# krea-ai/realtime-video

Hardware: AMD Instinct MI355X
Metric: frames/sec at 832x480, 4-step 14B T2V (per-step DiT latency in config) (higher is better)
Workload: dtype bf16

## Files before the change

realtime_video_amd/_lib.py:

```python
import ctypes
import os
import re
import subprocess

_HERE = os.path.dirname(os.path.abspath(__file__))
LIB_PATH = os.environ.get("RTV_LIB_PATH") or os.path.join(_HERE, "librtv_hip.so")
CSRC = os.path.join(_HERE, "csrc")

_INCLUDE = os.path.join(os.path.dirname(_HERE), "include")
HEADERS = ("rtv_hip.h", "rtv_hip_lab.h")

_lib = None

_SCALARS = {"int": ctypes.c_int, "int64_t": ctypes.c_int64, "float": ctypes.c_float, "double": ctypes.c_double,
            "size_t": ctypes.c_size_t}
_RETURNS = {"int": ctypes.c_int, "size_t": ctypes.c_size_t, "const char*": ctypes.c_char_p}
_STARS = r"(\*(?:\s*const\s*\*)?)?"


def _field_type(base, stars, structs):
    value = _SCALARS.get(base) or structs.get(base)
    if not stars:
        return value
    if base == "void":
        return ctypes.c_void_p if stars == "*" else ctypes.POINTER(ctypes.c_void_p)
    return ctypes.POINTER(value) if value and stars == "*" else None


def _param_type(base, stars, structs):
    if not stars:
        return ctypes.c_void_p if base == "rtv_stream_t" else _SCALARS.get(base)
    if base in structs:
        return ctypes.POINTER(structs[base]) if stars == "*" else None
    return ctypes.c_void_p if base == "void" or base in _SCALARS else None


def parse_header(text, structs):
    text = re.sub(r"/\*.*?\*/", "", text, flags=re.S)
    text = re.sub(r"#ifdef __cplusplus.*?#endif", "", text, flags=re.S)
    text = re.sub(r"^[ \t]*#.*$", "", text, flags=re.M)
    text = re.sub(r"\benum\s*\{[^}]*\}\s*;|\btypedef\s+void\s*\*\s*rtv_stream_t\s*;", "", text)

    def struct(m):
        name, fields = m.group(2), []
        for decl in filter(None, (d.strip() for d in m.group(1).split(";"))):
            head = re.match(r"(?:const\s+)?(\w+)\s*", decl)
            for item in decl[head.end():].split(","):
                d = re.fullmatch(_STARS + r"\s*(\w+)((?:\s*\[\d+\])*)", item.strip())
                t = d and _field_type(head.group(1), re.sub(r"\s", "", d.group(1) or ""), structs)
                if not t:
                    raise ValueError(f"{name}: cannot bind field declaration `{decl}`")
                for n in reversed(re.findall(r"\d+", d.group(3))):
                    t = t * int(n)
                fields.append((d.group(2), t))
        structs[name] = type(name, (ctypes.Structure,), {"_fields_": fields})
        return ""

    text = re.sub(r"\btypedef\s+struct\s*\w*\s*\{([^}]*)\}\s*(\w+)\s*;", struct, text)
    protos = {}
    for stmt in filter(None, (" ".join(s.split()) for s in text.split(";"))):
        m = re.fullmatch(r"(.*?)\s*\b(\w+)\s*\((.*)\)", stmt)
        if not m:
            raise ValueError(f"cannot bind declaration `{stmt}`")
        ret, name, params = m.group(1).replace(" *", "*"), m.group(2), m.group(3).strip()
        if ret not in _RETURNS:
            raise ValueError(f"{name}: cannot bind return type `{ret}`")
        argtypes = []
        for param in ([] if params == "void" else params.split(",")):
            d = re.fullmatch(r"(?:const\s+)?(\w+)\s*" + _STARS + r"\s*(\w+)?", param.strip())
            t = d and _param_type(d.group(1), re.sub(r"\s", "", d.group(2) or ""), structs)
            if not t:
                raise ValueError(f"{name}: cannot bind parameter `{param.strip()}`")
            argtypes.append(t)
        protos[name] = (_RETURNS[ret], argtypes)
    return protos


def _read(name):
    with open(os.path.join(_INCLUDE, name)) as f:
        return f.read()


STRUCTS, PROTOTYPES = {}, {}
for _name in HEADERS:
    PROTOTYPES.update(parse_header(_read(_name), STRUCTS))
IO_HEADER = "rtv_hip_io.h"
IO_STRUCTS = dict(STRUCTS)
IO_PROTOTYPES = parse_header(_read(IO_HEADER), IO_STRUCTS)
IO_STRUCTS = {k: v for k, v in IO_STRUCTS.items() if k not in STRUCTS}
JPEG_HEADER = "rtv_hip_jpeg.h"
JPEG_STRUCTS = dict(STRUCTS)
JPEG_PROTOTYPES = parse_header(_read(JPEG_HEADER), JPEG_STRUCTS)
JPEG_STRUCTS = {k: v for k, v in JPEG_STRUCTS.items() if k not in STRUCTS}
JPEGDEC_HEADER = "rtv_hip_jpeg_decode.h"
JPEGDEC_STRUCTS = dict(STRUCTS)
JPEGDEC_PROTOTYPES = parse_header(_read(JPEGDEC_HEADER), JPEGDEC_STRUCTS)
JPEGDEC_STRUCTS = {k: v for k, v in JPEGDEC_STRUCTS.items() if k not in STRUCTS}
LORA_HEADER = "rtv_hip_lora.h"
LORA_STRUCTS = dict(STRUCTS)
LORA_PROTOTYPES = parse_header(_read(LORA_HEADER), LORA_STRUCTS)
LORA_STRUCTS = {k: v for k, v in LORA_STRUCTS.items() if k not in STRUCTS}
CROSS_FOLD_HEADER = "rtv_hip_cross_fold.h"
CROSS_FOLD_STRUCTS = dict(STRUCTS)
CROSS_FOLD_PROTOTYPES = parse_header(_read(CROSS_FOLD_HEADER), CROSS_FOLD_STRUCTS)
FP8_ROWS_HEADER = "rtv_hip_fp8_rows.h"
FP8_ROWS_PROTOTYPES = parse_header(_read(FP8_ROWS_HEADER), dict(STRUCTS))
ATTN_FP8_HEADER = "rtv_hip_attn_fp8.h"
ATTN_FP8_STRUCTS = dict(STRUCTS)
ATTN_FP8_PROTOTYPES = parse_header(_read(ATTN_FP8_HEADER), ATTN_FP8_STRUCTS)
ATTN_FP8_STRUCTS = {k: v for k, v in ATTN_FP8_STRUCTS.items() if k not in STRUCTS}
MXFP4_HEADER = "rtv_hip_mxfp4.h"
MXFP4_PROTOTYPES = parse_header(_read(MXFP4_HEADER), dict(STRUCTS))
MXFP6_HEADER = "rtv_hip_mxfp6.h"
MXFP6_PROTOTYPES = parse_header(_read(MXFP6_HEADER), dict(STRUCTS))
MX_ROTATE_HEADER = "rtv_hip_mx_rotate.h"
MX_ROTATE_PROTOTYPES = parse_header(_read(MX_ROTATE_HEADER), dict(STRUCTS))
MX_ROT_ACT_SHIFT, MX_ROT_WEIGHT_SHIFT, MX_ROT_MAX_SHIFT = (
    int(re.search(rf"^#define\s+RTV_MX_ROT_{n}_SHIFT\s+(\d+)", _read(MX_ROTATE_HEADER), flags=re.M).group(1)) for n in ("ACT", "WEIGHT", "MAX"))
LORA_MAX_ADAPTERS, LORA_MAX_RANK = (int(re.search(rf"^#define\s+RTV_LORA_MAX_{n}\s+(\d+)", _read(LORA_HEADER), flags=re.M).group(1))
                                    for n in ("ADAPTERS", "RANK"))
FRAMES_MAX = int(re.search(r"^#define\s+RTV_FRAMES_MAX\s+(\d+)", _read(IO_HEADER), flags=re.M).group(1))
ABI_VERSION = int(re.search(r"^#define\s+RTV_ABI_VERSION\s+(\d+)", _read(HEADERS[0]), flags=re.M).group(1))


def build(verbose=False):
    jobs = os.environ.get("MAX_JOBS") or str(min(16, len(os.sched_getaffinity(0)) if hasattr(os, "sched_getaffinity") else os.cpu_count() or 4))
    cmd = ["make", "-C", CSRC, "-j", jobs]
    res = subprocess.run(cmd, capture_output=True, text=True)
    if verbose or res.returncode != 0:
        print(res.stdout[-4000:])
        print(res.stderr[-4000:])
    if res.returncode != 0:
        raise RuntimeError("building librtv_hip.so failed")
    return LIB_PATH


def declared_symbols(lab=True):
    out = set()
    for name in HEADERS if lab else HEADERS[:1]:
        text = re.sub(r"/\*.*?\*/", "", _read(name), flags=re.S)
        out.update(re.findall(r"\b(rtv_[a-z0-9_]+)\s*\(", text))
    return sorted(out)


def load():
    global _lib
    if _lib is not None:
        return _lib
    if not os.path.exists(LIB_PATH):
        raise RuntimeError(
            f"{LIB_PATH} is missing: run `python -c 'import __graft_entry__ as g; g.build()'` "
            "(or `make -C realtime_video_amd/csrc`). There is no CPU fallback for the HIP path.")
    lib = ctypes.CDLL(LIB_PATH)
    for name, (restype, argtypes) in list(PROTOTYPES.items()) + list(IO_PROTOTYPES.items()) + list(JPEG_PROTOTYPES.items()) + list(JPEGDEC_PROTOTYPES.items()) + list(LORA_PROTOTYPES.items()) + list(CROSS_FOLD_PROTOTYPES.items()) + list(FP8_ROWS_PROTOTYPES.items()) + list(ATTN_FP8_PROTOTYPES.items()) + list(MXFP4_PROTOTYPES.items()) + list(MXFP6_PROTOTYPES.items()) + list(MX_ROTATE_PROTOTYPES.items()):
        fn = getattr(lib, name, None)
        if fn is None:
            if os.environ.get("RTV_LIB_PATH"):
                continue
            raise RuntimeError(f"librtv_hip.so does not export {name}")
        fn.restype, fn.argtypes = restype, argtypes
    have = lib.rtv_version()
    if have != ABI_VERSION:
        raise RuntimeError(f"{LIB_PATH} reports ABI revision {have}, include/rtv_hip.h declares RTV_ABI_VERSION {ABI_VERSION}: "
                           "rebuild the library (`make -C realtime_video_amd/csrc`)")
    _lib = lib
    return lib


def check(status, what):
    if status != 0:
        msg = load().rtv_last_error().decode("utf-8", "replace")
        raise RuntimeError(f"{what} failed (status {status}): {msg}")


def call(name, *args):
    check(getattr(load(), name)(*args), name)
```

realtime_video_amd/csrc/vae_decode.hip:

```cpp
#include "gemm_core.h"
#include "rtv_internal.h"

namespace rtv {

struct ConvParams;
int launch_conv(const ConvParams& p, hipStream_t stream);

constexpr int RN_CHUNKS = 3;
__global__ __launch_bounds__(256) void rmsnorm_silu_cl_kernel(const f16_t* __restrict__ x, f16_t* __restrict__ out,
                                                             const f16_t* __restrict__ gamma, int C,
                                                             int64_t npix, int apply_silu) {
  __shared__ float ssq[64];
  __shared__ float part[256 * RN_CHUNKS];
  const int G = C >> 3;
  const int ppb = (256 * RN_CHUNKS) / G;
  const int64_t pix0 = (int64_t)blockIdx.x * ppb;
  float v[RN_CHUNKS][8];
  int lp[RN_CHUNKS];
#pragma unroll
  for (int i = 0; i < RN_CHUNKS; ++i) {
    const int c = threadIdx.x + i * 256;
    lp[i] = c / G;
    const int64_t pix = pix0 + lp[i];
    float s = 0.f;
    if (pix < npix) {
      u32x4 raw = *(const u32x4*)(x + pix * C + (c - lp[i] * G) * 8);
#pragma unroll
      for (int j = 0; j < 4; ++j) {
        const uint32_t u = raw[j];
        unpack_f16x2(u, v[i][2 * j], v[i][2 * j + 1]);
        s += v[i][2 * j] * v[i][2 * j] + v[i][2 * j + 1] * v[i][2 * j + 1];
      }
    }
    part[c] = s;
  }
  __syncthreads();
  if ((int)threadIdx.x < ppb) {
    float t = 0.f;
    for (int k = 0; k < G; ++k) t += part[threadIdx.x * G + k];
    ssq[threadIdx.x] = t;
  }
  __syncthreads();
  const float sqrtC = sqrtf((float)C);
#pragma unroll
  for (int i = 0; i < RN_CHUNKS; ++i) {
    const int c = threadIdx.x + i * 256;
    const int64_t pix = pix0 + lp[i];
    if (pix < npix) {
      const int ch = (c - lp[i] * G) * 8;
      const float inv = sqrtC / fmaxf(sqrtf(ssq[lp[i]]), 1e-12f);
      u32x4 graw = *(const u32x4*)(gamma + ch);
      u32x4 o;
#pragma unroll
      for (int j = 0; j < 4; ++j) {
        const uint32_t gu = graw[j];
        float g0, g1;
        unpack_f16x2(gu, g0, g1);
        float a = v[i][2 * j] * inv * g0;
        float b = v[i][2 * j + 1] * inv * g1;
        if (apply_silu) {
          a = silu(a);
          b = silu(b);
        }
        o[j] = pack_f16x2(a, b);
      }
      *(u32x4*)(out + pix * C + ch) = o;
    }
  }
}

__global__ __launch_bounds__(256) void softmax_rows_kernel(const f16_t* __restrict__ s, int lds_, f16_t* __restrict__ p,
                                                          int ldp, int n) {
  __shared__ float red[8];
  const int row = blockIdx.x;
  const f16_t* sr = s + (size_t)row * lds_;
  f16_t* pr = p + (size_t)row * ldp;
  float mx = -INFINITY;
  for (int c = threadIdx.x * 8; c < n; c += 256 * 8) {
    u32x4 raw = *(const u32x4*)(sr + c);
#pragma unroll
    for (int j = 0; j < 4; ++j) {
      const uint32_t u = raw[j];
      float a, b;
      unpack_f16x2(u, a, b);
      mx = fmaxf(mx, fmaxf(a, b));
    }
  }
  mx = wave_max(mx);
  if ((threadIdx.x & 63) == 0) red[threadIdx.x >> 6] = mx;
  __syncthreads();
  mx = fmaxf(fmaxf(red[0], red[1]), fmaxf(red[2], red[3]));
  float sum = 0.f;
  for (int c = threadIdx.x * 8; c < n; c += 256 * 8) {
    u32x4 raw = *(const u32x4*)(sr + c);
#pragma unroll
    for (int j = 0; j < 4; ++j) {
      const uint32_t u = raw[j];
      float a, b;
      unpack_f16x2(u, a, b);
      sum += __expf(a - mx) + __expf(b - mx);
    }
  }
  sum = wave_sum(sum);
  __syncthreads();
  if ((threadIdx.x & 63) == 0) red[4 + (threadIdx.x >> 6)] = sum;
  __syncthreads();
  const float inv = 1.0f / (red[4] + red[5] + red[6] + red[7]);
  for (int c = threadIdx.x * 8; c < ldp; c += 256 * 8) {
    u32x4 o = {0u, 0u, 0u, 0u};
    if (c < n) {
      u32x4 raw = *(const u32x4*)(sr + c);
#pragma unroll
      for (int j = 0; j < 4; ++j) {
        const uint32_t u = raw[j];
        float a, b;
        unpack_f16x2(u, a, b);
        o[j] = pack_f16x2(__expf(a - mx) * inv, __expf(b - mx) * inv);
      }
    }
    *(u32x4*)(pr + c) = o;
  }
}

__global__ void upsample_cache_t1_kernel(f16_t* buf, int64_t slice) {
  for (int64_t i = (int64_t)blockIdx.x * blockDim.x + threadIdx.x; i < slice; i += (int64_t)gridDim.x * blockDim.x) {
    f16_t c1 = buf[slice + i], x = buf[2 * slice + i];
    buf[i] = ((c1 & 0x7fff) == 0) ? (f16_t)0 : x;
    buf[slice + i] = x;
  }
}

__global__ void vae_prep_kernel(const f16_t* __restrict__ z, int t, int hw, const float* __restrict__ mean,
                                const float* __restrict__ stdv, const float* __restrict__ w2 ,
                                const float* __restrict__ b2, f16_t* __restrict__ out) {
  const int p = blockIdx.x * blockDim.x + threadIdx.x;
  if (p >= hw) return;
  float zin[16];
#pragma unroll
  for (int c = 0; c < 16; ++c) {
    float zz = f16_to_f32(z[((size_t)t * 16 + c) * hw + p]);
    float inv = round_f16(1.0f / round_f16(stdv[c]));
    zin[c] = round_f16(round_f16(zz / inv) + round_f16(mean[c]));
  }
  u32x4 o[4];
#pragma unroll
  for (int co = 0; co < 16; co += 2) {
    float a = b2[co], b = b2[co + 1];
#pragma unroll
    for (int c = 0; c < 16; ++c) {
      a += w2[co * 16 + c] * zin[c];
      b += w2[(co + 1) * 16 + c] * zin[c];
    }
    o[co >> 3][(co & 7) >> 1] = pack_f16x2(a, b);
  }
  o[2] = u32x4{0u, 0u, 0u, 0u};
  o[3] = u32x4{0u, 0u, 0u, 0u};
  u32x4* dst = (u32x4*)(out + (size_t)p * 32);
  dst[0] = o[0];
  dst[1] = o[1];
  dst[2] = o[2];
  dst[3] = o[3];
}

__global__ void vae_final_kernel(const f16_t* __restrict__ in, float* __restrict__ out, int T, int64_t hw, int64_t in_hw,
                                 int64_t skip_px) {
  const int64_t total = (int64_t)T * hw;
  for (int64_t i = (int64_t)blockIdx.x * blockDim.x + threadIdx.x; i < total; i += (int64_t)gridDim.x * blockDim.x) {
    const int64_t t = i / hw, p = i - t * hw;
    u32x2 raw = *(const u32x2*)(in + (t * in_hw + skip_px + p) * 8);
    const uint32_t u0 = raw[0], u1 = raw[1];
    float c0, c1, c2, c3;
    unpack_f16x2(u0, c0, c1);
    unpack_f16x2(u1, c2, c3);
    float r = fminf(fmaxf(c0, -1.f), 1.f), g = fminf(fmaxf(c1, -1.f), 1.f), bl = fminf(fmaxf(c2, -1.f), 1.f);
    out[(t * 3 + 0) * hw + p] = r;
    out[(t * 3 + 1) * hw + p] = g;
    out[(t * 3 + 2) * hw + p] = bl;
  }
}

}

using namespace rtv;

extern "C" int rtv_conv_cl(const void* in, const void* w, const void* bias, const void* residual, int res_ld,
                           void* out, int out_ld, int T, int H, int W, int Cin, int Cout, int kt, int kh, int kw,
                           int resample, int n_split, const void* zeros, rtv_stream_t stream);

#define RTV_TRY(expr)       \
  do {                      \
    int _s = (expr);        \
    if (_s != 0) return _s; \
  } while (0)

extern "C" int rtv_rmsnorm_silu_cl(const void* x, void* out, const void* gamma, int C, int64_t npix, int apply_silu,
                                   rtv_stream_t stream) {
  if (npix <= 0) return 0;
  if (C % 8 || 768 % (C / 8) || (768 / (C / 8)) > 64) return set_error(-1, "rmsnorm_silu_cl: C must be 96, 192, 384 (or another divisor layout of 768 chunks)");
  const int ppb = 768 / (C / 8);
  ProfScope prof(PROF_LN, (hipStream_t)stream, 2.0 * npix * C * 2);
  hipLaunchKernelGGL(rmsnorm_silu_cl_kernel, dim3((unsigned)((npix + ppb - 1) / ppb)), dim3(256), 0,
                     (hipStream_t)stream, (const f16_t*)x, (f16_t*)out, (const f16_t*)gamma, C, npix, apply_silu);
  return check_launch("rmsnorm_silu_cl");
}

extern "C" int rtv_softmax_rows(const void* s, int lds_, void* p, int ldp, int rows, int n, rtv_stream_t stream) {
  if (rows <= 0) return 0;
  if (n % 8 || lds_ % 8 || ldp % 8 || ldp < n) return set_error(-1, "softmax_rows: n / strides must be multiples of 8");
  hipLaunchKernelGGL(softmax_rows_kernel, dim3(rows), dim3(256), 0, (hipStream_t)stream, (const f16_t*)s, lds_,
                     (f16_t*)p, ldp, n);
  return check_launch("softmax_rows");
}

namespace {

struct Stage {
  int H, W;
};

struct RowPlan {
  int a[4], b[4];
  int r0, r1;
};

static int make_plan(int h, int r0, int r1, RowPlan* P) {
  const int H3 = h << 3;
  if (r0 < 0 || r1 > H3 || r0 >= r1) return set_error(-1, "vae_decode: bad pixel row range");
  P->r0 = r0;
  P->r1 = r1;
  P->a[3] = r0 - 7 > 0 ? r0 - 7 : 0;
  P->b[3] = r1 + 7 < H3 ? r1 + 7 : H3;
  for (int s = 2; s >= 1; --s) {
    const int Hs = h << s;
    int lo = (P->a[s + 1] - 1) >> 1, hi = (P->b[s + 1] >> 1) + 1;
    if (lo < 0) lo = 0;
    if (hi > Hs) hi = Hs;
    P->a[s] = lo - 6 > 0 ? lo - 6 : 0;
    P->b[s] = hi + 6 < Hs ? hi + 6 : Hs;
  }
  P->a[0] = 0;
  P->b[0] = h;
  return 0;
}

struct VaeLayout {
  size_t cat_off[32];
  int cat_C[32], cat_stage[32], cat_T[32];
  int cat_cap[32];
  size_t cat_slice[32];
  size_t act_off[4];
  size_t s_off, p_off, q_off, k_off, vt_off, o_off, xn_off;
  size_t head_off;
  size_t zeros_off;
  size_t total;
  int ldp;
};

template <class Take>
static void take_attn(VaeLayout* L, size_t P, Take&& take) {
  L->ldp = (int)((P + 63) / 64 * 64);
  L->s_off = take(P * P * 2);
  L->p_off = take(P * (size_t)L->ldp * 2);
  L->q_off = take(P * 384 * 2);
  L->k_off = take(P * 384 * 2);
  L->vt_off = take((size_t)384 * L->ldp * 2);
  L->o_off = take(P * 384 * 2);
  L->xn_off = take(P * 384 * 2);
}

constexpr int SLIDE_FRAMES = 3;

static void build_layout(int h, int w, const RowPlan& plan, VaeLayout* L) {
  const int C[32] = {32, 384, 384, 384, 384,
                     384, 384, 384, 384, 384, 384, 384,
                     192, 384, 384, 384, 384, 384, 384,
                     192, 192, 192, 192, 192, 192,
                     96, 96, 96, 96, 96, 96, 96};
  const int S[32] = {0, 0, 0, 0, 0, 0, 0, 0, 0, 0, 0, 0, 1, 1, 1, 1, 1, 1, 1, 2, 2, 2, 2, 2, 2, 3, 3, 3, 3, 3, 3, 3};
  const int Tm[4] = {1, 2, 4, 4};
  size_t off = 0;
  auto take = [&](size_t bytes) {
    size_t a = (off + 255) & ~(size_t)255;
    off = a + bytes;
    return a;
  };
  for (int i = 0; i < 32; ++i) {
    const int s = S[i];
    const size_t hw = (size_t)(plan.b[s] - plan.a[s]) * (w << s);
    L->cat_C[i] = C[i];
    L->cat_stage[i] = s;
    L->cat_T[i] = Tm[s];
    const bool time_conv_buf = i == 11 || i == 18;
    L->cat_cap[i] = 2 + (time_conv_buf ? 1 : SLIDE_FRAMES) * Tm[s];
    L->cat_slice[i] = hw * C[i] * 2;
    L->cat_off[i] = take((size_t)L->cat_cap[i] * L->cat_slice[i]);
  }
  size_t amax = 0;
  const int actC[4] = {768, 768, 384, 192};
  for (int s = 0; s < 4; ++s) {
    size_t hw = (size_t)(plan.b[s] - plan.a[s]) * (w << s);
    size_t b = (size_t)Tm[s] * hw * actC[s] * 2;
    if (b > amax) amax = b;
    if (s < 3) {
      size_t hw1 = (size_t)(plan.b[s + 1] - plan.a[s + 1]) * (w << (s + 1));
      size_t b1 = (size_t)Tm[s + 1] * hw1 * (actC[s] / 4) * 2;
      if (b1 > amax) amax = b1;
    }
  }
  for (int i = 0; i < 4; ++i) L->act_off[i] = take(amax);
  take_attn(L, (size_t)h * w, take);
  L->head_off = take((size_t)4 * (plan.b[3] - plan.a[3]) * (w << 3) * 8 * 2);
  L->zeros_off = take(256);
  L->total = off + 256;
}

}

extern "C" size_t rtv_vae_arena_bytes_rows(int h, int w, int row0, int row1) {
  if (h <= 0 || w <= 0) return 0;
  RowPlan P;
  if (make_plan(h, row0, row1, &P)) return 0;
  VaeLayout L;
  build_layout(h, w, P, &L);
  return L.total;
}

extern "C" size_t rtv_vae_arena_bytes(int h, int w) { return rtv_vae_arena_bytes_rows(h, w, 0, h << 3); }

extern "C" int rtv_vae_cache_slot_rows(int h, int w, int row0, int row1, int slot, size_t* offset, int* C, int* H,
                                       int* W, int* first_row) {
  if (slot < 0 || slot >= 32) return set_error(-1, "vae_cache_slot: slot out of range");
  RowPlan P;
  RTV_TRY(make_plan(h, row0, row1, &P));
  VaeLayout L;
  build_layout(h, w, P, &L);
  const int s = L.cat_stage[slot];
  *offset = L.cat_off[slot];
  *C = L.cat_C[slot];
  *H = P.b[s] - P.a[s];
  *W = w << s;
  *first_row = P.a[s];
  return 0;
}

extern "C" int rtv_vae_cache_slot(int h, int w, int slot, size_t* offset, int* C, int* H, int* W) {
  int first_row = 0;
  return rtv_vae_cache_slot_rows(h, w, 0, h << 3, slot, offset, C, H, W, &first_row);
}

namespace {

static std::atomic<bool> g_fresh_tap_skip{true};

struct Ctx {
  char* arena;
  const VaeLayout* L;
  int h, wd;
  hipStream_t stream;
  int act_next;
  bool fresh = false;
  int pos[32] = {};
  uint16_t* act(int i) { return (uint16_t*)(arena + L->act_off[i & 3]); }
  uint16_t* cat(int i) { return (uint16_t*)(arena + L->cat_off[i] + (size_t)pos[i] * L->cat_slice[i]); }
  const void* zeros() { return arena + L->zeros_off; }
};

static int roll_cache(Ctx& c, int ci, int T, int H, int W, int Cin);
static int cached_conv3(Ctx& c, int ci, int T, int H, int W, int Cin, const rtv_vae_conv& cw, int Cout,
                        const void* residual, void* out, int out_ld) {
  uint16_t* buf = c.cat(ci);
  const int flags = W == c.wd ? RTV_CONV_GATHER : RTV_CONV_NONE;
  if (c.fresh && T == 1) {
    RTV_TRY(conv3_last_tap(buf + 2 * (size_t)H * W * Cin, cw.w, cw.b, nullptr, residual, Cout, out, out_ld, H, W, Cin, Cout, flags,
                           c.zeros(), c.stream));
  } else {
    RTV_TRY(rtv_conv_cl(buf, cw.w, cw.b, residual, Cout, out, out_ld, T, H, W, Cin, Cout, 3, 3, 3, flags, 0, c.zeros(), c.stream));
  }
  return roll_cache(c, ci, T, H, W, Cin);
}

static int cache_to_front(Ctx& c, int ci, int from) {
  char* b = c.arena + c.L->cat_off[ci];
  const size_t slice = c.L->cat_slice[ci];
  c.pos[ci] = 0;
  if (from == 0) return 0;
  if (from == 1) {
    if (hipMemcpyAsync(b, b + slice, slice, hipMemcpyDeviceToDevice, c.stream) != hipSuccess ||
        hipMemcpyAsync(b + slice, b + 2 * slice, slice, hipMemcpyDeviceToDevice, c.stream) != hipSuccess)
      return set_error(-1, "vae: cache roll memcpy failed");
    return 0;
  }
  if (hipMemcpyAsync(b, b + (size_t)from * slice, 2 * slice, hipMemcpyDeviceToDevice, c.stream) != hipSuccess)
    return set_error(-1, "vae: cache roll memcpy failed");
  return 0;
}
static int roll_cache(Ctx& c, int ci, int T, int H, int W, int Cin) {
  if ((size_t)H * W * Cin * 2 != c.L->cat_slice[ci]) return set_error(-1, "vae: concat buffer geometry mismatch");
  const int np = c.pos[ci] + T;
  if (np + 2 + c.L->cat_T[ci] <= c.L->cat_cap[ci]) {
    c.pos[ci] = np;
    return 0;
  }
  return cache_to_front(c, ci, np);
}
static int flush_caches(Ctx& c, int n) {
  for (int i = 0; i < n; ++i)
    if (c.pos[i]) RTV_TRY(cache_to_front(c, i, c.pos[i]));
  return 0;
}

static int res_block(Ctx& c, int ci, int T, int H, int W, int cin, int cout, const rtv_vae_res& rw,
                     const uint16_t* x, uint16_t* tmp, uint16_t* sc_buf, uint16_t* y) {
  const int64_t npix = (int64_t)T * H * W;
  const size_t sl_in = (size_t)H * W * cin, sl_out = (size_t)H * W * cout;
  RTV_TRY(rtv_rmsnorm_silu_cl(x, c.cat(ci) + 2 * sl_in, rw.gamma0, cin, npix, 1, c.stream));
  {
    const int flags = W == c.wd ? RTV_CONV_GATHER : RTV_CONV_NONE;
    int st = cout != 96 ? 1
             : (c.fresh && T == 1)
                 ? conv3_last_tap(c.cat(ci) + 2 * sl_in, rw.conv_a.w, rw.conv_a.b, rw.gamma3, nullptr, 0, c.cat(ci + 1) + 2 * sl_out, cout,
                                  H, W, cin, cout, flags, c.zeros(), c.stream)
                 : rtv_conv3_norm_silu_cl(c.cat(ci), rw.conv_a.w, rw.conv_a.b, rw.gamma3, c.cat(ci + 1) + 2 * sl_out, cout, T, H, W, cin,
                                          cout, flags, c.zeros(), c.stream);
    if (st < 0) return st;
    if (st == 0) {
      RTV_TRY(roll_cache(c, ci, T, H, W, cin));
    } else {
      RTV_TRY(cached_conv3(c, ci, T, H, W, cin, rw.conv_a, cout, nullptr, tmp, cout));
      RTV_TRY(rtv_rmsnorm_silu_cl(tmp, c.cat(ci + 1) + 2 * sl_out, rw.gamma3, cout, npix, 1, c.stream));
    }
  }
  const uint16_t* hres = x;
  if (rw.shortcut.w) {
    if (cin % 64 == 0)
      RTV_TRY(rtv_gemm(x, cin, rw.shortcut.w, cin, sc_buf, cout, (int)npix, cout, cin, rw.shortcut.b, 0, nullptr, 0, 0, 0,
                       nullptr, 0, RTV_DTYPE_F16, 0, c.stream));
    else
      RTV_TRY(rtv_conv_cl(x, rw.shortcut.w, rw.shortcut.b, nullptr, 0, sc_buf, cout, T, H, W, cin, cout, 1, 1, 1, 0, 0,
                          c.zeros(), c.stream));
    hres = sc_buf;
  }
  RTV_TRY(cached_conv3(c, ci + 1, T, H, W, cout, rw.conv_b, cout, hres, y, cout));
  return 0;
}

static int mid_attention(Ctx& c, const rtv_vae_attn& a, const uint16_t* x, uint16_t* y) {
  const int P = c.h * c.wd, C = 384, ldp = c.L->ldp;
  char* A = c.arena;
  uint16_t *S = (uint16_t*)(A + c.L->s_off), *Pm = (uint16_t*)(A + c.L->p_off), *q = (uint16_t*)(A + c.L->q_off),
           *k = (uint16_t*)(A + c.L->k_off), *vt = (uint16_t*)(A + c.L->vt_off), *o = (uint16_t*)(A + c.L->o_off),
           *xn = (uint16_t*)(A + c.L->xn_off);
  auto G = [&](const void* a_, int lda, const void* w_, int ldw, void* out, int ldc, int M, int N, int K,
               const void* bias, const void* res, int ldr) {
    return rtv_gemm(a_, lda, w_, ldw, out, ldc, M, N, K, bias, 0, nullptr, 0, 0, 0, res, ldr, RTV_DTYPE_F16, 0, c.stream);
  };
  RTV_TRY(rtv_rmsnorm_silu_cl(x, xn, a.gamma, C, P, 0, c.stream));
  RTV_TRY(G(xn, C, a.wq, C, q, C, P, C, C, a.bq, nullptr, 0));
  RTV_TRY(G(xn, C, a.wk, C, k, C, P, C, C, a.bk, nullptr, 0));
  RTV_TRY(G(a.wv, C, xn, C, vt, ldp, C, P, C, nullptr, nullptr, 0));
  RTV_TRY(G(q, C, k, C, S, P, P, P, C, nullptr, nullptr, 0));
  RTV_TRY(rtv_softmax_rows(S, P, Pm, ldp, P, P, c.stream));
  RTV_TRY(G(Pm, ldp, vt, ldp, o, C, P, C, ldp, a.bv, nullptr, 0));
  RTV_TRY(G(o, C, a.wproj, C, y, C, P, C, C, a.bproj, x, C));
  return 0;
}

static bool clear_vt_pad(char* arena, const VaeLayout& L, int P, hipStream_t stream) {
  if (L.ldp == P) return true;
  return hipMemsetAsync(arena + L.vt_off, 0, (size_t)384 * L.ldp * 2, stream) == hipSuccess;
}

static int launch_vae_prep(const void* z, int t, int hw, const void* mean, const void* stdv, const void* w2, const void* b2,
                           void* out, hipStream_t stream) {
  hipLaunchKernelGGL(vae_prep_kernel, dim3((hw + 127) / 128), dim3(128), 0, stream, (const f16_t*)z, t, hw, (const float*)mean,
                     (const float*)stdv, (const float*)w2, (const float*)b2, (f16_t*)out);
  return check_launch("vae_prep");
}
static int launch_vae_final(const void* in, void* out, int T, int64_t hw, int64_t in_hw, int64_t skip_px, hipStream_t stream) {
  hipLaunchKernelGGL(vae_final_kernel, dim3(2048), dim3(256), 0, stream, (const f16_t*)in, (float*)out, T, hw, in_hw, skip_px);
  return check_launch("vae_final");
}
static int launch_upsample_cache_t1(void* buf, int64_t slice, hipStream_t stream) {
  hipLaunchKernelGGL(upsample_cache_t1_kernel, dim3(1024), dim3(256), 0, stream, (f16_t*)buf, slice);
  return check_launch("upsample_cache_t1");
}

}

extern "C" int rtv_conv_cl_win(const void* in, const void* w, const void* bias, const void* residual, int res_ld,
                               void* out, int out_ld, int T, int H, int W, int Cin, int Cout, int kt, int kh, int kw,
                               int resample, int n_split, const void* zeros, int y_out0, int y_in0, int in_rows,
                               int img_rows, rtv_stream_t stream);

static int vae_decode_impl(const rtv_vae_weights* w, const void* z, int T, int h, int wd, int first, int row0, int row1,
                           void* arena, size_t arena_bytes, void* pixels, rtv_stream_t stream_, bool single) {
  if (!w || !z || !arena || !pixels) return set_error(-1, "vae_decode: null argument");
  if (T <= 0) return 0;
  if ((h * wd) % 8) return set_error(-1, "vae_decode: h*w must be a multiple of 8");
  if (((uintptr_t)arena) & 255) return set_error(-1, "vae_decode: arena must be 256-byte aligned");
  RowPlan P;
  RTV_TRY(make_plan(h, row0, row1, &P));
  VaeLayout L;
  build_layout(h, wd, P, &L);
  if (arena_bytes < L.total) return set_error(-1, "vae_decode: arena too small (see rtv_vae_arena_bytes)");
  hipStream_t stream = (hipStream_t)stream_;
  Ctx c{(char*)arena, &L, h, wd, stream, 0};
  const int W8 = wd * 8;
  const int64_t out_hw = (int64_t)(row1 - row0) * W8;
  int out_frame = 0;
  if (!clear_vt_pad((char*)arena, L, h * wd, stream)) return set_error(-1, "vae_decode: memset failed");

  for (int f = 0; f < T; ++f) {
    const bool is_first = first && f == 0;
    int H = h, W = wd, Tn = 1;
    uint16_t *a0 = c.act(0), *a1 = c.act(1), *a2 = c.act(2), *a3 = c.act(3);
    {
      const size_t sl = (size_t)H * W * 32;
      RTV_TRY(launch_vae_prep(z, f, H * W, w->mean, w->std, w->conv2_w, w->conv2_b, c.cat(0) + 2 * sl, stream));
    }
    RTV_TRY(cached_conv3(c, 0, 1, H, W, 32, w->conv1, 384, nullptr, a0, 384));
    RTV_TRY(res_block(c, 1, 1, H, W, 384, 384, w->mid0, a0, a1, a2, a3));
    RTV_TRY(mid_attention(c, w->attn, a3, a0));
    RTV_TRY(res_block(c, 3, 1, H, W, 384, 384, w->mid2, a0, a1, a2, a3));
    uint16_t* x = a3;
    int ci = 5;
    for (int s = 0; s < 4; ++s) {
      const int cout = (s == 0 || s == 1) ? 384 : (s == 2 ? 192 : 96);
      int cin = (s == 0) ? 384 : (s == 1 ? 192 : (s == 2 ? 192 : 96));
      for (int r = 0; r < 3; ++r) {
        uint16_t* bufs[3];
        int nb = 0;
        for (int i = 0; i < 4; ++i)
          if (c.act(i) != x) bufs[nb++] = c.act(i);
        RTV_TRY(res_block(c, ci, Tn, H, W, cin, cout, w->up[s * 3 + r], x, bufs[0], bufs[1], bufs[2]));
        x = bufs[2];
        ci += 2;
        cin = cout;
      }
      if (s == 3) break;
      uint16_t* free_[3];
      int nb = 0;
      for (int i = 0; i < 4; ++i)
        if (c.act(i) != x) free_[nb++] = c.act(i);
      if (s < 2) {
        const size_t sl = (size_t)H * W * cout;
        uint16_t* buf = c.cat(ci);
        if (is_first && single) {
          for (int t = 0; t < Tn; ++t) {
            if (hipMemsetAsync(free_[0] + (size_t)(2 * t) * sl, 0, sl * 2, stream) != hipSuccess ||
                hipMemcpyAsync(free_[0] + (size_t)(2 * t + 1) * sl, x + (size_t)t * sl, sl * 2, hipMemcpyDeviceToDevice, stream) !=
                    hipSuccess)
              return set_error(-1, "vae_decode: memset / memcpy failed");
          }
          x = free_[0];
          Tn *= 2;
          nb = 0;
          for (int i = 0; i < 4; ++i)
            if (c.act(i) != x) free_[nb++] = c.act(i);
        } else if (!is_first) {
          if (hipMemcpyAsync(buf + 2 * sl, x, (size_t)Tn * sl * 2, hipMemcpyDeviceToDevice, stream) != hipSuccess)
            return set_error(-1, "vae_decode: memcpy failed");
          RTV_TRY(rtv_conv_cl(buf, w->time_conv[s].w, w->time_conv[s].b, nullptr, 0, free_[0], cout, Tn, H, W, cout,
                              2 * cout, 3, 1, 1, 0, cout, c.zeros(), stream));
          if (Tn == 1 && single) {
            if (hipMemsetAsync(buf, 0, sl * 2, stream) != hipSuccess ||
                hipMemcpyAsync(buf + sl, buf + 2 * sl, sl * 2, hipMemcpyDeviceToDevice, stream) != hipSuccess)
              return set_error(-1, "vae_decode: memset / memcpy failed");
          } else if (Tn == 1) {
            RTV_TRY(launch_upsample_cache_t1(buf, (int64_t)sl, stream));
          } else {
            if (hipMemcpyAsync(buf, buf + (size_t)Tn * sl, 2 * sl * 2, hipMemcpyDeviceToDevice, stream) != hipSuccess)
              return set_error(-1, "vae_decode: memcpy failed");
          }
          x = free_[0];
          Tn *= 2;
          nb = 0;
          for (int i = 0; i < 4; ++i)
            if (c.act(i) != x) free_[nb++] = c.act(i);
        }
        ci += 1;
      }
      const int Hn = P.b[s + 1] - P.a[s + 1];
      RTV_TRY(rtv_conv_cl_win(x, w->resample[s].w, w->resample[s].b, nullptr, 0, free_[0], cout / 2, Tn, Hn, 2 * W, cout,
                              cout / 2, 1, 3, 3, RTV_CONV_UPSAMPLE2X, 0, c.zeros(), P.a[s + 1], P.a[s], H, h << (s + 1),
                              stream));
      x = free_[0];
      H = Hn;
      W *= 2;
    }
    {
      const size_t sl = (size_t)H * W * 96;
      RTV_TRY(rtv_rmsnorm_silu_cl(x, c.cat(31) + 2 * sl, w->head_gamma, 96, (int64_t)Tn * H * W, 1, stream));
      uint16_t* ho = (uint16_t*)((char*)arena + L.head_off);
      RTV_TRY(cached_conv3(c, 31, Tn, H, W, 96, w->head, 8, nullptr, ho, 8));
      RTV_TRY(launch_vae_final(ho, (float*)pixels + (size_t)out_frame * 3 * out_hw, Tn, out_hw, (int64_t)H * W,
                               (int64_t)(row0 - P.a[3]) * W, stream));
      out_frame += Tn;
    }
  }
  return flush_caches(c, 32);
}

extern "C" int rtv_vae_decode_rows(const rtv_vae_weights* w, const void* z, int T, int h, int wd, int first, int row0,
                                   int row1, void* arena, size_t arena_bytes, void* pixels, rtv_stream_t stream) {
  return vae_decode_impl(w, z, T, h, wd, first, row0, row1, arena, arena_bytes, pixels, stream, false);
}

extern "C" int rtv_vae_decode(const rtv_vae_weights* w, const void* z, int T, int h, int wd, int first, void* arena,
                              size_t arena_bytes, void* pixels, rtv_stream_t stream) {
  return vae_decode_impl(w, z, T, h, wd, first, 0, h << 3, arena, arena_bytes, pixels, stream, false);
}

extern "C" int rtv_vae_decode_single(const rtv_vae_weights* w, const void* z, int h, int wd, int is_first_frame, void* arena,
                                     size_t arena_bytes, void* pixels, rtv_stream_t stream) {
  return vae_decode_impl(w, z, 1, h, wd, is_first_frame ? 1 : 0, 0, h << 3, arena, arena_bytes, pixels, stream, true);
}

static bool aligned16(const void* p) { return (((uintptr_t)p) & 15) == 0; }

extern "C" size_t rtv_vae_attn_arena_bytes(int h, int w) {
  if (h <= 0 || w <= 0 || (int64_t)h * w > (1 << 20) || (h * w) % 8) return 0;
  VaeLayout L;
  size_t off = 0;
  take_attn(&L, (size_t)h * w, [&](size_t bytes) {
    size_t a = (off + 255) & ~(size_t)255;
    off = a + bytes;
    return a;
  });
  return off + 256;
}

extern "C" int rtv_vae_mid_attention(const rtv_vae_attn* a, const void* x, void* y, int h, int w, void* arena,
                                     size_t arena_bytes, rtv_stream_t stream_) {
  if (!a || !x || !y || !arena) return set_error(-1, "vae_mid_attention: null argument");
  if (!a->gamma || !a->wq || !a->bq || !a->wk || !a->bk || !a->wv || !a->bv || !a->wproj || !a->bproj)
    return set_error(-1, "vae_mid_attention: null weight");
  if (x == y) return set_error(-1, "vae_mid_attention: x and y must be different buffers (x is the residual)");
  if (h <= 0 || w <= 0 || (int64_t)h * w > (1 << 20) || (h * w) % 8)
    return set_error(-1, "vae_mid_attention: h*w must be a positive multiple of 8");
  if ((((uintptr_t)arena) & 255) || !aligned16(x) || !aligned16(y))
    return set_error(-1, "vae_mid_attention: arena must be 256-byte aligned, x / y 16-byte aligned");
  VaeLayout L;
  size_t off = 0;
  take_attn(&L, (size_t)h * w, [&](size_t bytes) {
    size_t at = (off + 255) & ~(size_t)255;
    off = at + bytes;
    return at;
  });
  L.total = off + 256;
  if (arena_bytes < L.total) return set_error(-1, "vae_mid_attention: arena too small (see rtv_vae_attn_arena_bytes)");
  hipStream_t stream = (hipStream_t)stream_;
  Ctx c{(char*)arena, &L, h, w, stream, 0};
  if (!clear_vt_pad((char*)arena, L, h * w, stream)) return set_error(-1, "vae_mid_attention: memset failed");
  return mid_attention(c, *a, (const uint16_t*)x, (uint16_t*)y);
}

extern "C" int rtv_vae_prep(const void* z, int T, int t, int hw, const void* mean, const void* stdv, const void* conv2_w,
                            const void* conv2_b, void* out, rtv_stream_t stream) {
  if (!z || !mean || !stdv || !conv2_w || !conv2_b || !out) return set_error(-1, "vae_prep: null argument");
  if (T <= 0 || t < 0 || t >= T || hw <= 0 || hw > (1 << 24)) return set_error(-1, "vae_prep: frame index or size out of range");
  if (!aligned16(out)) return set_error(-1, "vae_prep: out must be 16-byte aligned");
  return launch_vae_prep(z, t, hw, mean, stdv, conv2_w, conv2_b, out, (hipStream_t)stream);
}

extern "C" int rtv_vae_final(const void* in, void* pixels, int T, int64_t hw, int64_t in_hw, int64_t skip_px,
                             rtv_stream_t stream) {
  if (!in || !pixels) return set_error(-1, "vae_final: null argument");
  if (T <= 0 || hw <= 0 || skip_px < 0 || skip_px + hw > in_hw || in_hw > ((int64_t)1 << 32) / T)
    return set_error(-1, "vae_final: the row window [skip_px, skip_px + hw) must lie inside a frame of in_hw pixels");
  if (!aligned16(in)) return set_error(-1, "vae_final: in must be 16-byte aligned");
  return launch_vae_final(in, pixels, T, hw, in_hw, skip_px, (hipStream_t)stream);
}

extern "C" int rtv_vae_upsample_cache_t1(void* buf, int64_t slice, rtv_stream_t stream) {
  if (!buf) return set_error(-1, "vae_upsample_cache_t1: null argument");
  if (slice <= 0 || slice > ((int64_t)1 << 32)) return set_error(-1, "vae_upsample_cache_t1: slice must be positive");
  return launch_upsample_cache_t1(buf, slice, (hipStream_t)stream);
}

namespace rtv {

__global__ void vae_enc_prep_kernel(const f16_t* __restrict__ frames, int Ttot, int t0, int T, int64_t hw,
                                    f16_t* __restrict__ out) {
  const int64_t total = (int64_t)T * hw;
  for (int64_t i = (int64_t)blockIdx.x * blockDim.x + threadIdx.x; i < total; i += (int64_t)gridDim.x * blockDim.x) {
    const int64_t t = i / hw, p = i - t * hw;
    const f16_t r = frames[((int64_t)0 * Ttot + t0 + t) * hw + p];
    const f16_t g = frames[((int64_t)1 * Ttot + t0 + t) * hw + p];
    const f16_t b = frames[((int64_t)2 * Ttot + t0 + t) * hw + p];
    u32x4* dst = (u32x4*)(out + i * 32);
    dst[0] = u32x4{(uint32_t)r | ((uint32_t)g << 16), (uint32_t)b, 0u, 0u};
    dst[1] = u32x4{0u, 0u, 0u, 0u};
    dst[2] = u32x4{0u, 0u, 0u, 0u};
    dst[3] = u32x4{0u, 0u, 0u, 0u};
  }
}

__global__ void vae_enc_final_kernel(const f16_t* __restrict__ in, int T, int64_t hw, const float* __restrict__ w1 ,
                                     const float* __restrict__ b1, const float* __restrict__ mean,
                                     const float* __restrict__ stdv, f16_t* __restrict__ mu, int Tout_tot, int tout) {
  const int64_t total = (int64_t)T * hw;
  const int64_t i = (int64_t)blockIdx.x * blockDim.x + threadIdx.x;
  if (i >= total) return;
  const int64_t t = i / hw, p = i - t * hw;
  float x[32];
  const u32x4* src = (const u32x4*)(in + i * 32);
#pragma unroll
  for (int q = 0; q < 4; ++q) {
    u32x4 raw = src[q];
#pragma unroll
    for (int j = 0; j < 4; ++j) {
      const uint32_t u = raw[j];
      unpack_f16x2(u, x[q * 8 + 2 * j], x[q * 8 + 2 * j + 1]);
    }
  }
#pragma unroll 4
  for (int co = 0; co < 16; ++co) {
    float a = b1[co];
#pragma unroll
    for (int c = 0; c < 32; ++c) a += w1[co * 32 + c] * x[c];
    const float inv = round_f16(1.0f / round_f16(stdv[co]));
    const float v = round_f16(round_f16(round_f16(a) - round_f16(mean[co])) * inv);
    mu[((int64_t)co * Tout_tot + tout + t) * hw + p] = f32_to_f16(v);
  }
}

}

namespace {

static int launch_vae_enc_prep(const void* frames, int Ttot, int t0, int T, int64_t hw, void* out, hipStream_t stream) {
  hipLaunchKernelGGL(vae_enc_prep_kernel, dim3(2048), dim3(256), 0, stream, (const f16_t*)frames, Ttot, t0, T, hw, (f16_t*)out);
  return check_launch("vae_enc_prep");
}
static int launch_vae_enc_final(const void* in, int T, int64_t hw, const void* w1, const void* b1, const void* mean,
                                const void* stdv, void* mu, int Tout_tot, int tout, hipStream_t stream) {
  hipLaunchKernelGGL(vae_enc_final_kernel, dim3((unsigned)((T * hw + 127) / 128)), dim3(128), 0, stream, (const f16_t*)in, T, hw,
                     (const float*)w1, (const float*)b1, (const float*)mean, (const float*)stdv, (f16_t*)mu, Tout_tot, tout);
  return check_launch("vae_enc_final");
}

static void build_enc_layout(int H, int W, VaeLayout* L) {
  const int C[24] = {32, 96, 96, 96, 96,
                     96, 192, 192, 192, 192,
                     192, 384, 384, 384, 384,
                     384, 384, 384, 384,
                     384, 384, 384, 384, 384};
  const int S[24] = {0, 0, 0, 0, 0, 1, 1, 1, 1, 2, 2, 2, 2, 2, 3, 3, 3, 3, 3, 3, 3, 3, 3, 3};
  const int Tm[24] = {4, 4, 4, 4, 4, 4, 4, 4, 4, 4, 2, 2, 2, 2, 2, 1, 1, 1, 1, 1, 1, 1, 1, 1};
  size_t off = 0;
  auto take = [&](size_t bytes) {
    size_t a = (off + 255) & ~(size_t)255;
    off = a + bytes;
// ... 173 lines not shown
```

Baseline: 19.36.

## Batch multiple latent frames per VAE decode pass

The VAE decoder now processes up to three latent frames together through the conv and resblock stages instead of one frame per iteration. Causal time-conv caches and the upsample time conv stay per-frame. The arena layout grows its activation and head buffers to hold the group, and a group size is picked so the conv kernel selection stays the same. The aim is larger conv launches with better GPU use and fewer launches, at the cost of a larger arena and more complex cache rolling.

New measurement: 19.47, median of 6. No clear change (+0.6%).

```diff
diff --git a/include/rtv_hip_vae_group.h b/include/rtv_hip_vae_group.h
--- /dev/null
+++ b/include/rtv_hip_vae_group.h
@@ -0,0 +1,18 @@
+#ifndef RTV_HIP_VAE_GROUP_H
+#define RTV_HIP_VAE_GROUP_H
+#include "rtv_hip.h"
+
+#ifdef __cplusplus
+extern "C" {
+#endif
+
+int rtv_vae_set_group_frames(int g);
+
+int rtv_vae_group_frames(int h, int w, int row0, int row1);
+
+size_t rtv_vae_arena_bytes_group(int h, int w, int row0, int row1, int g);
+
+#ifdef __cplusplus
+}
+#endif
+#endif
diff --git a/realtime_video_amd/_lib.py b/realtime_video_amd/_lib.py
--- a/realtime_video_amd/_lib.py
+++ b/realtime_video_amd/_lib.py
@@ -115,6 +115,8 @@
 MXFP6_PROTOTYPES = parse_header(_read(MXFP6_HEADER), dict(STRUCTS))
 MX_ROTATE_HEADER = "rtv_hip_mx_rotate.h"
 MX_ROTATE_PROTOTYPES = parse_header(_read(MX_ROTATE_HEADER), dict(STRUCTS))
+VAE_GROUP_HEADER = "rtv_hip_vae_group.h"
+VAE_GROUP_PROTOTYPES = parse_header(_read(VAE_GROUP_HEADER), dict(STRUCTS))
 MX_ROT_ACT_SHIFT, MX_ROT_WEIGHT_SHIFT, MX_ROT_MAX_SHIFT = (
     int(re.search(rf"^#define\s+RTV_MX_ROT_{n}_SHIFT\s+(\d+)", _read(MX_ROTATE_HEADER), flags=re.M).group(1)) for n in ("ACT", "WEIGHT", "MAX"))
 LORA_MAX_ADAPTERS, LORA_MAX_RANK = (int(re.search(rf"^#define\s+RTV_LORA_MAX_{n}\s+(\d+)", _read(LORA_HEADER), flags=re.M).group(1))
@@ -152,7 +154,7 @@
             f"{LIB_PATH} is missing: run `python -c 'import __graft_entry__ as g; g.build()'` "
             "(or `make -C realtime_video_amd/csrc`). There is no CPU fallback for the HIP path.")
     lib = ctypes.CDLL(LIB_PATH)
-    for name, (restype, argtypes) in list(PROTOTYPES.items()) + list(IO_PROTOTYPES.items()) + list(JPEG_PROTOTYPES.items()) + list(JPEGDEC_PROTOTYPES.items()) + list(LORA_PROTOTYPES.items()) + list(CROSS_FOLD_PROTOTYPES.items()) + list(FP8_ROWS_PROTOTYPES.items()) + list(ATTN_FP8_PROTOTYPES.items()) + list(MXFP4_PROTOTYPES.items()) + list(MXFP6_PROTOTYPES.items()) + list(MX_ROTATE_PROTOTYPES.items()):
+    for name, (restype, argtypes) in list(PROTOTYPES.items()) + list(IO_PROTOTYPES.items()) + list(JPEG_PROTOTYPES.items()) + list(JPEGDEC_PROTOTYPES.items()) + list(LORA_PROTOTYPES.items()) + list(CROSS_FOLD_PROTOTYPES.items()) + list(FP8_ROWS_PROTOTYPES.items()) + list(ATTN_FP8_PROTOTYPES.items()) + list(MXFP4_PROTOTYPES.items()) + list(MXFP6_PROTOTYPES.items()) + list(MX_ROTATE_PROTOTYPES.items()) + list(VAE_GROUP_PROTOTYPES.items()):
         fn = getattr(lib, name, None)
         if fn is None:
             if os.environ.get("RTV_LIB_PATH"):
diff --git a/realtime_video_amd/csrc/vae_decode.hip b/realtime_video_amd/csrc/vae_decode.hip
--- a/realtime_video_amd/csrc/vae_decode.hip
+++ b/realtime_video_amd/csrc/vae_decode.hip
@@ -1,5 +1,6 @@
 #include "gemm_core.h"
 #include "rtv_internal.h"
+#include "../../include/rtv_hip_vae_group.h"
 
 namespace rtv {
 
@@ -254,6 +255,7 @@
   size_t zeros_off;
   size_t total;
   int ldp;
+  int group;
 };
 
 template <class Take>
@@ -270,14 +272,40 @@
 
 constexpr int SLIDE_FRAMES = 3;
 
-static void build_layout(int h, int w, const RowPlan& plan, VaeLayout* L) {
-  const int C[32] = {32, 384, 384, 384, 384,
-                     384, 384, 384, 384, 384, 384, 384,
-                     192, 384, 384, 384, 384, 384, 384,
-                     192, 192, 192, 192, 192, 192,
-                     96, 96, 96, 96, 96, 96, 96};
-  const int S[32] = {0, 0, 0, 0, 0, 0, 0, 0, 0, 0, 0, 0, 1, 1, 1, 1, 1, 1, 1, 2, 2, 2, 2, 2, 2, 3, 3, 3, 3, 3, 3, 3};
-  const int Tm[4] = {1, 2, 4, 4};
+constexpr int DEC_C[32] = {32, 384, 384, 384, 384,
+                           384, 384, 384, 384, 384, 384, 384,
+                           192, 384, 384, 384, 384, 384, 384,
+                           192, 192, 192, 192, 192, 192,
+                           96, 96, 96, 96, 96, 96, 96};
+constexpr int DEC_S[32] = {0, 0, 0, 0, 0, 0, 0, 0, 0, 0, 0, 0, 1, 1, 1, 1, 1, 1, 1, 2, 2, 2, 2, 2, 2, 3, 3, 3, 3, 3, 3, 3};
+constexpr int DEC_TM[4] = {1, 2, 4, 4};
+constexpr int DEC_WIDTH[4] = {384, 384, 192, 96};
+static bool is_time_conv_buf(int i) { return i == 11 || i == 18; }
+
+static bool same_kernels(size_t hw, int C, int T1, int Tg) {
+  const size_t e1 = (size_t)(T1 + 2) * hw * C, eg = (size_t)(Tg + 2) * hw * C;
+  return (e1 >= 0x40000000ull) == (eg >= 0x40000000ull) && (e1 >= 0x7fffffffull) == (eg >= 0x7fffffffull);
+}
+static int pick_group(int w, const RowPlan& plan) {
+  for (int g = SLIDE_FRAMES; g > 1; --g) {
+    bool ok = true;
+    for (int i = 0; i < 32 && ok; ++i) {
+      const int s = DEC_S[i];
+      if (!is_time_conv_buf(i))
+        ok = same_kernels((size_t)(plan.b[s] - plan.a[s]) * (w << s), DEC_C[i], DEC_TM[s], g * DEC_TM[s]);
+    }
+    for (int s = 0; s < 3 && ok; ++s)
+      ok = same_kernels((size_t)(plan.b[s] - plan.a[s]) * (w << s), DEC_WIDTH[s], DEC_TM[s + 1], g * DEC_TM[s + 1]);
+    if (ok) return g;
+  }
+  return 1;
+}
+
+static void build_layout(int h, int w, const RowPlan& plan, VaeLayout* L, int group = 0) {
+  const int* C = DEC_C;
+  const int* S = DEC_S;
+  const int* Tm = DEC_TM;
+  L->group = group > 0 ? group : pick_group(w, plan);
   size_t off = 0;
   auto take = [&](size_t bytes) {
     size_t a = (off + 255) & ~(size_t)255;
@@ -290,26 +318,24 @@
     L->cat_C[i] = C[i];
     L->cat_stage[i] = s;
     L->cat_T[i] = Tm[s];
-    const bool time_conv_buf = i == 11 || i == 18;
-    L->cat_cap[i] = 2 + (time_conv_buf ? 1 : SLIDE_FRAMES) * Tm[s];
+    L->cat_cap[i] = 2 + (is_time_conv_buf(i) ? 1 : SLIDE_FRAMES) * Tm[s];
     L->cat_slice[i] = hw * C[i] * 2;
     L->cat_off[i] = take((size_t)L->cat_cap[i] * L->cat_slice[i]);
   }
   size_t amax = 0;
-  const int actC[4] = {768, 768, 384, 192};
   for (int s = 0; s < 4; ++s) {
     size_t hw = (size_t)(plan.b[s] - plan.a[s]) * (w << s);
-    size_t b = (size_t)Tm[s] * hw * actC[s] * 2;
+    size_t b = (size_t)L->group * Tm[s] * (s < 2 ? 2 : 1) * hw * DEC_WIDTH[s] * 2;
     if (b > amax) amax = b;
     if (s < 3) {
       size_t hw1 = (size_t)(plan.b[s + 1] - plan.a[s + 1]) * (w << (s + 1));
-      size_t b1 = (size_t)Tm[s + 1] * hw1 * (actC[s] / 4) * 2;
+      size_t b1 = (size_t)L->group * Tm[s + 1] * hw1 * (DEC_WIDTH[s] / 2) * 2;
       if (b1 > amax) amax = b1;
     }
   }
   for (int i = 0; i < 4; ++i) L->act_off[i] = take(amax);
   take_attn(L, (size_t)h * w, take);
-  L->head_off = take((size_t)4 * (plan.b[3] - plan.a[3]) * (w << 3) * 8 * 2);
+  L->head_off = take((size_t)L->group * Tm[3] * (plan.b[3] - plan.a[3]) * (w << 3) * 8 * 2);
   L->zeros_off = take(256);
   L->total = off + 256;
 }
@@ -326,6 +352,20 @@
 }
 
 extern "C" size_t rtv_vae_arena_bytes(int h, int w) { return rtv_vae_arena_bytes_rows(h, w, 0, h << 3); }
+
+extern "C" int rtv_vae_group_frames(int h, int w, int row0, int row1) {
+  RowPlan P;
+  if (h <= 0 || w <= 0 || make_plan(h, row0, row1, &P)) return 0;
+  return pick_group(w, P);
+}
+
+extern "C" size_t rtv_vae_arena_bytes_group(int h, int w, int row0, int row1, int g) {
+  RowPlan P;
+  if (h <= 0 || w <= 0 || g < 1 || g > SLIDE_FRAMES || make_plan(h, row0, row1, &P)) return 0;
+  VaeLayout L;
+  build_layout(h, w, P, &L, g);
+  return L.total;
+}
 
 extern "C" int rtv_vae_cache_slot_rows(int h, int w, int row0, int row1, int slot, size_t* offset, int* C, int* H,
                                        int* W, int* first_row) {
@@ -351,6 +391,7 @@
 namespace {
 
 static std::atomic<bool> g_fresh_tap_skip{true};
+static std::atomic<int> g_group_frames{0};
 
 struct Ctx {
   char* arena;
@@ -359,6 +400,7 @@
   hipStream_t stream;
   int act_next;
   bool fresh = false;
+  int group = 1;
   int pos[32] = {};
   uint16_t* act(int i) { return (uint16_t*)(arena + L->act_off[i & 3]); }
   uint16_t* cat(int i) { return (uint16_t*)(arena + L->cat_off[i] + (size_t)pos[i] * L->cat_slice[i]); }
@@ -397,7 +439,7 @@
 static int roll_cache(Ctx& c, int ci, int T, int H, int W, int Cin) {
   if ((size_t)H * W * Cin * 2 != c.L->cat_slice[ci]) return set_error(-1, "vae: concat buffer geometry mismatch");
   const int np = c.pos[ci] + T;
-  if (np + 2 + c.L->cat_T[ci] <= c.L->cat_cap[ci]) {
+  if (np + 2 + c.group * c.L->cat_T[ci] <= c.L->cat_cap[ci]) {
     c.pos[ci] = np;
     return 0;
   }
@@ -505,23 +547,27 @@
   if (arena_bytes < L.total) return set_error(-1, "vae_decode: arena too small (see rtv_vae_arena_bytes)");
   hipStream_t stream = (hipStream_t)stream_;
   Ctx c{(char*)arena, &L, h, wd, stream, 0};
+  const int want = g_group_frames.load(std::memory_order_relaxed);
+  c.group = want > 0 && want < L.group ? want : L.group;
   const int W8 = wd * 8;
   const int64_t out_hw = (int64_t)(row1 - row0) * W8;
   int out_frame = 0;
   if (!clear_vt_pad((char*)arena, L, h * wd, stream)) return set_error(-1, "vae_decode: memset failed");
 
-  for (int f = 0; f < T; ++f) {
+  for (int f = 0, g = 1; f < T; f += g) {
     const bool is_first = first && f == 0;
-    int H = h, W = wd, Tn = 1;
+    g = is_first ? 1 : (T - f < c.group ? T - f : c.group);
+    int H = h, W = wd, Tn = g;
     uint16_t *a0 = c.act(0), *a1 = c.act(1), *a2 = c.act(2), *a3 = c.act(3);
     {
       const size_t sl = (size_t)H * W * 32;
-      RTV_TRY(launch_vae_prep(z, f, H * W, w->mean, w->std, w->conv2_w, w->conv2_b, c.cat(0) + 2 * sl, stream));
-    }
-    RTV_TRY(cached_conv3(c, 0, 1, H, W, 32, w->conv1, 384, nullptr, a0, 384));
-    RTV_TRY(res_block(c, 1, 1, H, W, 384, 384, w->mid0, a0, a1, a2, a3));
-    RTV_TRY(mid_attention(c, w->attn, a3, a0));
-    RTV_TRY(res_block(c, 3, 1, H, W, 384, 384, w->mid2, a0, a1, a2, a3));
+      for (int j = 0; j < g; ++j)
+        RTV_TRY(launch_vae_prep(z, f + j, H * W, w->mean, w->std, w->conv2_w, w->conv2_b, c.cat(0) + (2 + j) * sl, stream));
+    }
+    RTV_TRY(cached_conv3(c, 0, g, H, W, 32, w->conv1, 384, nullptr, a0, 384));
+    RTV_TRY(res_block(c, 1, g, H, W, 384, 384, w->mid0, a0, a1, a2, a3));
+    for (int j = 0; j < g; ++j) RTV_TRY(mid_attention(c, w->attn, a3 + (size_t)j * H * W * 384, a0 + (size_t)j * H * W * 384));
+    RTV_TRY(res_block(c, 3, g, H, W, 384, 384, w->mid2, a0, a1, a2, a3));
     uint16_t* x = a3;
     int ci = 5;
     for (int s = 0; s < 4; ++s) {
@@ -558,19 +604,22 @@
           for (int i = 0; i < 4; ++i)
             if (c.act(i) != x) free_[nb++] = c.act(i);
         } else if (!is_first) {
-          if (hipMemcpyAsync(buf + 2 * sl, x, (size_t)Tn * sl * 2, hipMemcpyDeviceToDevice, stream) != hipSuccess)
-            return set_error(-1, "vae_decode: memcpy failed");
-          RTV_TRY(rtv_conv_cl(buf, w->time_conv[s].w, w->time_conv[s].b, nullptr, 0, free_[0], cout, Tn, H, W, cout,
-                              2 * cout, 3, 1, 1, 0, cout, c.zeros(), stream));
-          if (Tn == 1 && single) {
-            if (hipMemsetAsync(buf, 0, sl * 2, stream) != hipSuccess ||
-                hipMemcpyAsync(buf + sl, buf + 2 * sl, sl * 2, hipMemcpyDeviceToDevice, stream) != hipSuccess)
-              return set_error(-1, "vae_decode: memset / memcpy failed");
-          } else if (Tn == 1) {
-            RTV_TRY(launch_upsample_cache_t1(buf, (int64_t)sl, stream));
-          } else {
-            if (hipMemcpyAsync(buf, buf + (size_t)Tn * sl, 2 * sl * 2, hipMemcpyDeviceToDevice, stream) != hipSuccess)
+          const int Tf = Tn / g;
+          for (int j = 0; j < g; ++j) {
+            if (hipMemcpyAsync(buf + 2 * sl, x + (size_t)j * Tf * sl, (size_t)Tf * sl * 2, hipMemcpyDeviceToDevice, stream) != hipSuccess)
               return set_error(-1, "vae_decode: memcpy failed");
+            RTV_TRY(rtv_conv_cl(buf, w->time_conv[s].w, w->time_conv[s].b, nullptr, 0, free_[0] + (size_t)j * 2 * Tf * sl, cout, Tf, H, W,
+                                cout, 2 * cout, 3, 1, 1, 0, cout, c.zeros(), stream));
+            if (Tf == 1 && single) {
+              if (hipMemsetAsync(buf, 0, sl * 2, stream) != hipSuccess ||
+                  hipMemcpyAsync(buf + sl, buf + 2 * sl, sl * 2, hipMemcpyDeviceToDevice, stream) != hipSuccess)
+                return set_error(-1, "vae_decode: memset / memcpy failed");
+            } else if (Tf == 1) {
+              RTV_TRY(launch_upsample_cache_t1(buf, (int64_t)sl, stream));
+            } else {
+              if (hipMemcpyAsync(buf, buf + (size_t)Tf * sl, 2 * sl * 2, hipMemcpyDeviceToDevice, stream) != hipSuccess)
+                return set_error(-1, "vae_decode: memcpy failed");
+            }
           }
           x = free_[0];
           Tn *= 2;
@@ -599,6 +648,12 @@
     }
   }
   return flush_caches(c, 32);
+}
+
+extern "C" int rtv_vae_set_group_frames(int g) {
+  if (g < 0 || g > SLIDE_FRAMES) return set_error(-1, "vae_set_group_frames: 0 (default) .. 3 latent frames per group");
+  g_group_frames.store(g, std::memory_order_relaxed);
+  return 0;
 }
 
 extern "C" int rtv_vae_decode_rows(const rtv_vae_weights* w, const void* z, int T, int h, int wd, int first, int row0,
```
